# wei-zeng98/piano-a2s

Measured on AMD Instinct MI355X. Metric: training clips/sec (12 s, 5-bar), higher is better.
Workload: dtype f32

## Files before the change

piano_a2s_amd/csrc/a2s_api.hip:

```cpp
#include "a2s_common.h"
#include "../../include/a2s.h"

thread_local char a2s_err_msg[512] = {0};
long long a2s_launch_counter = 0;

int a2s_gemm_impl(hipStream_t, int, int, int, float, const float*, long, long, const float*, long, long, float, float*, long,
                  const float*, int, int, long, long, long, int, float*, size_t);
size_t a2s_gemm_workspace_bytes_impl(int, int, int, int);
int a2s_gemm_affine_impl(hipStream_t, int, int, int, float, const float*, long, long, const float*, long, long, float, float*, long, const float*,
                         int, int, long, long, long, int, float*, size_t, const float*, const float*, int, const float*, const float*, int,
                         const float*, const float*, const float*, const float*, const float*, float*, int, int, const float*, const float*);
int a2s_absmax_impl(hipStream_t, const float*, long, float*);
void a2s_gemm_f16x2_set(int);
int a2s_gemm_f16x2_enabled(void);
int a2s_gemm_bnstats_slots(int);
int a2s_conv3x3_impl(hipStream_t, const float*, const float*, float*, const float*, const float*, float*, int, int, int, int, int, int, float*,
                     const float*, const float*, const float*, const float*, const float*, const float*, const float*, float*);
void a2s_conv_rows_set(int);
void a2s_conv_c1_fast_set(int);
int a2s_conv_c1_fast_enabled(void);
int a2s_conv_rows_enabled(void);
void a2s_wgrad_rows_set(int);
int a2s_wgrad_rows_enabled(void);
void a2s_staff_emb_fast_set(int);
int a2s_staff_emb_fast_enabled(void);
void a2s_conv_f16x2_set(int);
int a2s_conv_f16x2_enabled(void);
size_t a2s_conv3x3_workspace_floats_impl(int);
void a2s_conv_bf16x3_set(int);
void a2s_gemm_split_set(int);
void a2s_wgrad_split_set(int);
int a2s_wgrad_split_enabled(void);
int a2s_gemm_split_enabled(void);
int a2s_conv_bf16x3_enabled(void);
int a2s_conv3x3_stat_blocks_impl(int, int, int, int);
int a2s_bn_finalize_impl(hipStream_t, const float*, int, int, double, const float*, const float*, float*, float*, long long*,
// ... 194 lines not shown
    if (!strcmp(key, "attn_deep")) { a2s_attn_deep_set(value); return A2S_OK; }
    if (!strcmp(key, "attn_defer_combine")) { a2s_attn_defer_combine_set(value); return A2S_OK; }
    if (!strcmp(key, "dec_mid")) { a2s_dec_mid_set(value); return A2S_OK; }
    if (!strcmp(key, "attn_pair")) { a2s_attn_pair_set(value); return A2S_OK; }
    if (!strcmp(key, "attn_pair_fused_rows")) { a2s_attn_pair_fused_rows_set(value); return A2S_OK; }
    if (!strcmp(key, "dec_fused_max_rows")) { a2s_dec_fused_max_rows_set(value); return A2S_OK; }
    if (!strcmp(key, "gru_fused")) { a2s_gru_step_fused_set(value); return A2S_OK; }
    if (!strcmp(key, "gru_persist")) { a2s_gru_persist_set(value); return A2S_OK; }
    if (!strcmp(key, "gru_persist_alone")) { a2s_gru_persist_alone_set(value); return A2S_OK; }
    if (!strcmp(key, "dec_persist")) { a2s_dec_persist_set(value); return A2S_OK; }
    if (!strcmp(key, "persist_force_agent")) { a2s_persist_dbg_set(PERSIST_DBG_FORCE_AGENT, value); return A2S_OK; }
    if (!strcmp(key, "persist_inject_abort")) { a2s_persist_dbg_set(PERSIST_DBG_INJECT_ABORT, value); return A2S_OK; }
    if (!strcmp(key, "gemm_tile")) { a2s_gemm_debug_tile_impl(value); return A2S_OK; }
    if (!strcmp(key, "conv_bf16x3")) { a2s_conv_bf16x3_set(value); return A2S_OK; }
    if (!strcmp(key, "conv_rows")) { a2s_conv_rows_set(value); return A2S_OK; }
    if (!strcmp(key, "conv_c1_fast")) { a2s_conv_c1_fast_set(value); return A2S_OK; }
    if (!strcmp(key, "wgrad_rows")) { a2s_wgrad_rows_set(value); return A2S_OK; }
    if (!strcmp(key, "staff_emb_fast")) { a2s_staff_emb_fast_set(value); return A2S_OK; }
    if (!strcmp(key, "conv_f16x2")) { a2s_conv_f16x2_set(value); return A2S_OK; }
    if (!strcmp(key, "wgrad_f16x2")) { a2s_wgrad_f16x2_set(value); return A2S_OK; }
    if (!strcmp(key, "gemm_bf16x3")) { a2s_gemm_split_set(value); return A2S_OK; }
    if (!strcmp(key, "gemm_f16x2")) { a2s_gemm_f16x2_set(value); return A2S_OK; }
    if (!strcmp(key, "wgrad_bf16x3")) { a2s_wgrad_split_set(value); return A2S_OK; }
    snprintf(a2s_err_msg, sizeof(a2s_err_msg), "a2s_debug_set: unknown key %s", key);
    return A2S_ERR_ARG;
}

int a2s_persist_abort_latch(void* device_word) { a2s_persist_latch_set(device_word); return A2S_OK; }

int a2s_debug_get(const char* key) {
    if (key && !strcmp(key, "attn_bulk_cap")) return a2s_attn_bulk_cap_enabled();
    if (key && !strcmp(key, "attn_deep")) return a2s_attn_deep_max_clips();
    if (key && !strcmp(key, "attn_defer_combine")) return a2s_attn_defer_combine_enabled();
    if (key && !strcmp(key, "dec_mid")) return a2s_dec_mid_enabled();
    if (key && !strcmp(key, "attn_pair")) return a2s_attn_pair_enabled();
    if (key && !strcmp(key, "attn_pair_fused_rows")) return a2s_attn_pair_fused_rows();
    if (key && !strcmp(key, "attn_pair_launches")) return (int)a2s_attn_pair_launches();
    if (key && !strcmp(key, "attn_pair_bwd_launches")) return (int)a2s_attn_pair_bwd_launches();
    if (key && !strcmp(key, "dec_mid_launches")) return a2s_dec_mid_launches();
    if (key && !strcmp(key, "conv_bf16x3")) return a2s_conv_bf16x3_enabled();
    if (key && !strcmp(key, "conv_rows")) return a2s_conv_rows_enabled();
    if (key && !strcmp(key, "conv_c1_fast")) return a2s_conv_c1_fast_enabled();
    if (key && !strcmp(key, "wgrad_rows")) return a2s_wgrad_rows_enabled();
    if (key && !strcmp(key, "staff_emb_fast")) return a2s_staff_emb_fast_enabled();
    if (key && !strcmp(key, "conv_f16x2")) return a2s_conv_f16x2_enabled();
    if (key && !strcmp(key, "wgrad_f16x2")) return a2s_wgrad_f16x2_enabled();
    if (key && !strcmp(key, "gemm_bf16x3")) return a2s_gemm_split_enabled();
    if (key && !strcmp(key, "gemm_f16x2")) return a2s_gemm_f16x2_enabled();
    if (key && !strcmp(key, "wgrad_bf16x3")) return a2s_wgrad_split_enabled();
    if (key && !strcmp(key, "gru_fused")) return a2s_gru_step_fused_enabled();
    if (key && !strcmp(key, "gru_persist")) return a2s_gru_persist_enabled();
    if (key && !strcmp(key, "gru_persist_alone")) return a2s_gru_persist_alone();
    if (key && !strcmp(key, "dec_persist")) return a2s_dec_persist_enabled();
    if (key && !strcmp(key, "dec_persist_launches")) return a2s_dec_persist_launches();
    if (key && !strcmp(key, "persist_force_agent")) return a2s_persist_dbg_get(PERSIST_DBG_FORCE_AGENT);
    if (key && !strcmp(key, "persist_inject_abort")) return a2s_persist_dbg_get(PERSIST_DBG_INJECT_ABORT);
// ... 254 lines not shown
```

piano_a2s_amd/csrc/a2s_conv_rows.hip:

```cpp
#include "a2s_common.h"
#include <type_traits>

#define RW_P 120
#define RW_SROW 288
#define RW_SLOTS 5
#ifndef RW_EB
#define RW_EB 4
#endif
#define RW_HDR 160

typedef short s16x4 __attribute__((ext_vector_type(4)));
typedef short s16x8 __attribute__((ext_vector_type(8)));
#define RW_LDS(p) ((__attribute__((address_space(3))) s16x4*)(p))

template <int CIN>
struct RwGeom {
    static constexpr int NB = CIN / 4;
    static constexpr int KS = (3 * NB + 7) / 8;
    static constexpr int TS = CIN * RW_SROW;
    static constexpr int SLOT = 2 * TS + (CIN % 8 ? 128 : 0);
    static constexpr int ITEMS = CIN * 32;
    static constexpr int XIT = (ITEMS + 255) / 256;
};

// ... 452 lines not shown
        const int grp = tid / (NJ * 5), c = tid % (NJ * 5);
        const float s = red[grp][c][0] + red[grp + 4][c][0], s2 = red[grp][c][1] + red[grp + 4][c][1];
        const float m = fmaxf(red[grp][c][2], red[grp + 4][c][2]);
        if (a.stat_partial) {
            a.stat_partial[((long)blockIdx.x * COUT + tid) * 2 + 0] = s;
            a.stat_partial[((long)blockIdx.x * COUT + tid) * 2 + 1] = s2;
        }
        if (a.out_absmax) {
            const unsigned bits = __float_as_uint(m);
            if (bits > __hip_atomic_load(reinterpret_cast<unsigned*>(a.out_absmax + tid), __ATOMIC_RELAXED, __HIP_MEMORY_SCOPE_AGENT))
                atomicMax(reinterpret_cast<unsigned*>(a.out_absmax + tid), bits);
        }
    }
}

template <int CIN, int COUT>
__global__ __launch_bounds__(256) void rows16_pack(const float* __restrict__ w, int flip, const float* __restrict__ in_scale,
                                                   const float* __restrict__ in_shift, const float* __restrict__ in_absmax,
                                                   const float* __restrict__ x_absmax, unsigned char* __restrict__ wimg, float* __restrict__ hdr,
                                                   float* __restrict__ out_absmax) {
    static_assert(COUT == 40, "rows16: 40 output channels");
    using G = RwGeom<CIN>;
    __shared__ int kci[CIN];
    __shared__ float red[16];
    __shared__ int kw[16];
    const int tile = blockIdx.x, tid = threadIdx.x;
    auto column = [&](int li, int& co, int& df) {
        if (tile < 6) { co = (tile / 3) * 16 + li; df = tile % 3; }
        else if (tile == 6) { co = 32 + (li & 7); df = li >> 3; }
        else { co = li < 8 ? 32 + li : -1; df = 2; }
    };
    if (tid < CIN) {
        int k = 0;
        if (in_scale) k = pow2_scale_exp(fabsf(in_scale[tid]) * (in_absmax ? in_absmax[tid] : 1.f) + fabsf(in_shift[tid]), 14);
        kci[tid] = k;
        if (tile == 0) {
            hdr[tid] = in_scale ? ldexpf(in_scale[tid], k) : 1.f;
            hdr[40 + tid] = in_scale ? ldexpf(in_shift[tid], k) : 0.f;
        }
    }
    if (tile == 0 && tid == 0) hdr[120] = ldexpf(1.f, (!in_scale && x_absmax) ? pow2_scale_exp(*x_absmax, 14) : 0);
    if (tile == 0 && out_absmax && tid < COUT) out_absmax[tid] = 0.f;
    __syncthreads();
// ... 21 lines not shown
        int co, df;
        column(li, co, df);
        float v = 0.f;
        if (co >= 0 && kb < 3 * G::NB) v = ldexpf(weight(co, 4 * (kb % G::NB) + e, (kb / G::NB) * 3 + df), kw[li]);
        unsigned t0, t1;
        split2_pair_f16(v, 0.f, t0, t1);
        unsigned short* dst = reinterpret_cast<unsigned short*>(wimg + ((size_t)(tile * G::KS + s) * 2) * 1024 + lane * 16 + e8 * 2);
        dst[0] = (unsigned short)t0;
        dst[512] = (unsigned short)t1;
    }
}

__device__ __forceinline__ float rw_ror8(float x) {
    return __int_as_float(__builtin_amdgcn_update_dpp(0, __float_as_int(x), 0x128, 0xf, 0xf, true));
}

#define R16_SLOTS 4
template <int CIN, int COUT, bool AFFINE, bool BNRED, bool PIPE = false>
__global__ __launch_bounds__(512, 2) void conv3x3_rows16(RowsArgs a) {
    static_assert(COUT == 40, "rows16: 40 output channels");
    using G = RwGeom<CIN>;
    constexpr int NTHR = 512, KS = G::KS;
    constexpr int XIT = (G::ITEMS + NTHR - 1) / NTHR;
    __shared__ __attribute__((aligned(16))) unsigned char ring[R16_SLOTS * G::SLOT];
    __shared__ __attribute__((aligned(16))) unsigned char b1img[PIPE ? 8 * G::KS * 1024 : 16];
    __shared__ float xch[2][5][2][16];
    __shared__ float red[8][16][3];
    __shared__ float tab[(AFFINE ? 2 * CIN : 0) + (BNRED ? 4 * COUT : 0) + 4];
    __shared__ __attribute__((aligned(16))) unsigned char dump[(G::ITEMS % NTHR) ? NTHR * 16 : 16];

    const int tid = threadIdx.x, lane = tid & 63;
    const int wave = __builtin_amdgcn_readfirstlane(tid >> 6);
    const int q = lane & 15, g = lane >> 4;
    const bool wide = wave < 4;
    const int m0 = wide ? 4 * (wave & 1) : 2 * (wave - 4);
    const int nm = wide ? 4 : 2;
    const int tile0 = wide ? 3 * (wave >> 1) : 6;
    const bool neg = wave & 1;
    const float sg = neg ? -1.f : 1.f;
    const int bnd_l = wide ? (wave & 1 ? (wave >> 1) : -1) : (wave > 4 ? wave - 3 : -1);
    const int bnd_r = wide ? (wave & 1 ? -1 : (wave >> 1)) : (wave < 7 ? wave - 2 : -1);

    int bid = blockIdx.x;
    {
        const int per = (int)gridDim.x / 8;
        if (bid < per * 8) bid = (bid % 8) * per + bid / 8;
    }
    const int ft = bid % a.tilesF; bid /= a.tilesF;
    const int strip = bid % a.nstrips, b = bid / a.nstrips;
    const int f_base = ft * RW_P;
    const int t_lo = strip * a.strip_len, t_hi = min(a.T, t_lo + a.strip_len);

    const unsigned sgn = neg ? 0x80008000u : 0u;
    constexpr int BWT = PIPE ? 1 : 2;
    s16x8 bw[3][KS][BWT];
#pragma unroll
    for (int d = 0; d < 3; ++d)
#pragma unroll
        for (int s = 0; s < KS; ++s)
#pragma unroll
            for (int tm = 0; tm < BWT; ++tm) {
                uint4 v = *reinterpret_cast<const uint4*>(a.wimg + ((size_t)((tile0 + ((wide || d < 2) ? d : 0)) * KS + s) * 2 + tm) * 1024 + lane * 16);
                v.x ^= sgn; v.y ^= sgn; v.z ^= sgn; v.w ^= sgn;
                bw[d][s][tm] = __builtin_bit_cast(s16x8, v);
            }
    if (PIPE) {
        for (int e = tid; e < 8 * KS * 64; e += NTHR)
            *reinterpret_cast<uint4*>(b1img + (size_t)e * 16) = *reinterpret_cast<const uint4*>(a.wimg + ((size_t)(e >> 6) * 2 + 1) * 1024 + (e & 63) * 16);
    }
    auto bterm1 = [&](int d, int s) -> s16x8 {
        if (PIPE) {
            uint4 v = *reinterpret_cast<const uint4*>(b1img + ((tile0 + ((wide || d < 2) ? d : 0)) * KS + s) * 1024 + lane * 16);
            v.x ^= sgn; v.y ^= sgn; v.z ^= sgn; v.w ^= sgn;
            return __builtin_bit_cast(s16x8, v);
        }
        return bw[d][s][BWT - 1];
    };
    const int co = wide ? (wave >> 1) * 16 + q : 32 + (q & 7);
    const bool useful = wide || q < 8;
    const float xscale = a.hdr[120];
    const float unsc = useful ? a.hdr[80 + co] / xscale * sg : 0.f;
    if (AFFINE && tid < 2 * CIN) tab[tid] = a.hdr[tid < CIN ? tid : 40 + tid - CIN];
    if (BNRED && tid < 4 * COUT) {
        const float* src = tid < COUT ? a.yl_mean : tid < 2 * COUT ? a.yl_invstd : tid < 3 * COUT ? a.yl_scale : a.yl_shift;
        tab[tid] = src[tid % COUT];
    }
    __syncthreads();
    float bm = 0.f, bi = 0.f, bsc = 0.f, bsh = 0.f;
    if (BNRED && useful) { bm = tab[co]; bi = tab[COUT + co]; bsc = tab[2 * COUT + co]; bsh = tab[3 * COUT + co]; }
    f32x2 st_s = {0.f, 0.f}, st_s2 = {0.f, 0.f};
    float st_m = 0.f;

    unsigned aaddr[KS][2];
#pragma unroll
// ... 43 lines not shown
        *reinterpret_cast<uint2*>(p0) = t0;
        *reinterpret_cast<uint2*>(p1) = t1;
    };

    f32x4 acc[4][3];
    auto multiply = [&](auto NMc, auto NTc, int crow, int cslot, const f32x4 (&xr)[XIT]) {
        constexpr int NM = decltype(NMc)::value, NT = decltype(NTc)::value;
        const bool cok = crow >= 0 && crow < a.T && colok;
        unsigned char* const cbase = ring + cslot * G::SLOT;
#pragma unroll
        for (int i = 0; i < NM; ++i)
#pragma unroll
            for (int d = 0; d < NT; ++d) acc[i][d] = (f32x4){0.f, 0.f, 0.f, 0.f};
#pragma unroll
        for (int s = 0; s < KS; ++s) {
#pragma unroll
            for (int ig = 0; ig < NM / 2; ++ig) {
                s16x8 av[2][2];
#pragma unroll
                for (int tm = 0; tm < 2; ++tm)
#pragma unroll
                    for (int ii = 0; ii < 2; ++ii) {
                        const int off = tm * G::TS + (ig * 2 + ii) * 32;
                        const s16x4 lo = __builtin_amdgcn_ds_read_tr16_b64_v4i16(RW_LDS(ring + aaddr[s][0] + off));
                        const s16x4 hi = __builtin_amdgcn_ds_read_tr16_b64_v4i16(RW_LDS(ring + aaddr[s][1] + off));
                        av[tm][ii] = __builtin_shufflevector(lo, hi, 0, 1, 2, 3, 4, 5, 6, 7);
                    }
#define R16_PRODUCT(TA, TB)                                                                                                  \
    _Pragma("unroll") for (int d = 0; d < NT; ++d)                                                                           \
        _Pragma("unroll") for (int ii = 0; ii < 2; ++ii)                                                                     \
            acc[ig * 2 + ii][d] = __builtin_amdgcn_mfma_f32_16x16x32_f16(__builtin_bit_cast(f16x8, av[TA][ii]), __builtin_bit_cast(f16x8, bw[d][s][TB < BWT ? TB : 0]), acc[ig * 2 + ii][d], 0, 0, 0);
                R16_PRODUCT(1, 0)
                R16_PRODUCT(0, 1)
                R16_PRODUCT(0, 0)
#undef R16_PRODUCT
            }
#pragma unroll
            for (int it = 0; it < XIT; ++it)
                if (it * KS / XIT == s) commit_item(it, cok, cbase, xr[it]);
        }
    };
    auto advance = [&]() {
#pragma unroll
        for (int s = 0; s < KS; ++s)
#pragma unroll
            for (int r = 0; r < 2; ++r) {
                const unsigned n = aaddr[s][r] + G::SLOT;
                aaddr[s][r] = min(n, n - R16_SLOTS * G::SLOT);
            }
    };

    const int up_addr = (((g + 3) & 3) * 16 + q) * 4;
    const int dn_addr = (((g + 1) & 3) * 16 + q) * 4;
    unsigned okbits = 0;
#pragma unroll
    for (int i = 0; i < 4; ++i) {
        const int p = 16 * (m0 + i) + 4 * g;
        if (useful && i < nm && p >= 4 && p < 4 + RW_P && f_base - 4 + p < a.F) okbits |= 1u << i;
    }
    const __amdgpu_buffer_rsrc_t yrsrc = __builtin_amdgcn_make_buffer_rsrc(a.y + (long)b * a.T * COUT * a.F, 0, (unsigned)((long)a.T * COUT * a.F * 4), 0x00020000);
    const __amdgpu_buffer_rsrc_t ylrsrc = __builtin_amdgcn_make_buffer_rsrc(const_cast<float*>(BNRED ? a.yl + (long)b * a.T * COUT * a.F : a.x), 0,
                                                                            BNRED ? (unsigned)((long)a.T * COUT * a.F * 4) : 0u, 0x00020000);
    const int yvo = (co * a.F + f_base - 4 + 16 * m0 + 4 * g) * 4;
    f32x4 ylv[BNRED ? 4 : 1];
    auto yl_fetch = [&](int t) {
        if (!BNRED) return;
        const int yrow_off = t * COUT * a.F * 4;
#pragma unroll
        for (int i = 0; i < 4; ++i)
            if (i < nm) ylv[BNRED ? i : 0] = __builtin_bit_cast(f32x4, __builtin_amdgcn_raw_buffer_load_b128(ylrsrc, yvo + 64 * i, yrow_off, 0));
    };
    auto epilogue = [&](auto WIDEc, int t, int par) {
        constexpr bool WIDE = decltype(WIDEc)::value;
        constexpr int NM = WIDE ? 4 : 2, D2 = WIDE ? 2 : 1;
        const int yrow_off = t * COUT * a.F * 4;
        const float xl = bnd_l >= 0 ? xch[par][bnd_l >= 0 ? bnd_l : 0][0][q] * sg : 0.f;
        const float xr_ = bnd_r >= 0 ? xch[par][bnd_r >= 0 ? bnd_r : 0][1][q] * sg : 0.f;
        unsigned ob = okbits;
        asm volatile("" : "+v"(ob));
        float X[NM], Y[NM];
#pragma unroll
        for (int i = 0; i < NM; ++i) {
            const float up_src = (g == 3) ? (i > 0 ? acc[i > 0 ? i - 1 : 0][0][3] : xl) : acc[i][0][3];
            const float dn_src = (g == 0) ? (i < NM - 1 ? acc[i < NM - 1 ? i + 1 : NM - 1][D2][0] : xr_) : acc[i][D2][0];
            X[i] = __int_as_float(__builtin_amdgcn_ds_bpermute(up_addr, __float_as_int(up_src)));
            Y[i] = __int_as_float(__builtin_amdgcn_ds_bpermute(dn_addr, __float_as_int(dn_src)));
        }
#pragma unroll
        for (int i = 0; i < NM; ++i) {
            const bool ok = ob >> i & 1;
            const float us = ok ? unsc : 0.f;
            f32x4 d1;
#pragma unroll
            for (int r = 0; r < 4; ++r) d1[r] = WIDE ? acc[i][1][r] : rw_ror8(acc[i][0][r]);
            f32x4 o;
            o[0] = ((X[i] + d1[0]) + acc[i][D2][1]) * us;
            o[1] = ((acc[i][0][0] + d1[1]) + acc[i][D2][2]) * us;
            o[2] = ((acc[i][0][1] + d1[2]) + acc[i][D2][3]) * us;
            o[3] = ((acc[i][0][2] + d1[3]) + Y[i]) * us;
            if (ok) __builtin_amdgcn_raw_buffer_store_b128(__builtin_bit_cast(u32x4, o), yrsrc, yvo + 64 * i, yrow_off, 0);
            if (BNRED) {
                const f32x4 xv = ylv[BNRED ? i : 0];
                f32x4 gm, xh;
#pragma unroll
                for (int k = 0; k < 4; ++k) {
                    gm[k] = (fmaf(xv[k], bsc, bsh) > 0.f) ? o[k] : 0.f;
                    xh[k] = fmaf(xv[k], bi, -bm * bi);
                }
                st_s += (f32x2){gm[0], gm[1]}; st_s += (f32x2){gm[2], gm[3]};
                st_s2 += (f32x2){gm[0], gm[1]} * (f32x2){xh[0], xh[1]}; st_s2 += (f32x2){gm[2], gm[3]} * (f32x2){xh[2], xh[3]};
                if (a.out_absmax) st_m = fmaxf(fmaxf(st_m, fmaxf(fabsf(o[0]), fabsf(o[1]))), fmaxf(fabsf(o[2]), fabsf(o[3])));
            } else {
                st_s += (f32x2){o[0], o[1]}; st_s += (f32x2){o[2], o[3]};
// ... 14 lines not shown
    __syncthreads();

    if constexpr (PIPE) {
        f32x4 accp[2][4][3];
#pragma unroll
        for (int e = 0; e < 2; ++e)
#pragma unroll
            for (int i = 0; i < 4; ++i)
#pragma unroll
                for (int d = 0; d < 3; ++d) accp[e][i][d] = (f32x4){0.f, 0.f, 0.f, 0.f};
        auto yl_tile = [&](int i, int t) -> f32x4 {
            return __builtin_bit_cast(f32x4, __builtin_amdgcn_raw_buffer_load_b128(ylrsrc, yvo + 64 * i, t * COUT * a.F * 4, 0));
        };
        auto epi_tile = [&](auto WIDEc, auto SETc, int i, int t, float xl, float xr_, unsigned ob, const f32x4& ylt) {
            constexpr bool WIDE = decltype(WIDEc)::value;
            constexpr int SET = decltype(SETc)::value, NM = WIDE ? 4 : 2, D2 = WIDE ? 2 : 1;
            const int yrow_off = t * COUT * a.F * 4;
            const float up_src = (g == 3) ? (i > 0 ? accp[SET][i > 0 ? i - 1 : 0][0][3] : xl) : accp[SET][i][0][3];
            const float dn_src = (g == 0) ? (i < NM - 1 ? accp[SET][i < NM - 1 ? i + 1 : NM - 1][D2][0] : xr_) : accp[SET][i][D2][0];
            const float X = __int_as_float(__builtin_amdgcn_ds_bpermute(up_addr, __float_as_int(up_src)));
            const float Y = __int_as_float(__builtin_amdgcn_ds_bpermute(dn_addr, __float_as_int(dn_src)));
            const bool ok = ob >> i & 1;
            const float us = ok ? unsc : 0.f;
            f32x4 d1;
#pragma unroll
            for (int r = 0; r < 4; ++r) d1[r] = WIDE ? accp[SET][i][1][r] : rw_ror8(accp[SET][i][0][r]);
            f32x4 o;
            o[0] = ((X + d1[0]) + accp[SET][i][D2][1]) * us;
            o[1] = ((accp[SET][i][0][0] + d1[1]) + accp[SET][i][D2][2]) * us;
            o[2] = ((accp[SET][i][0][1] + d1[2]) + accp[SET][i][D2][3]) * us;
            o[3] = ((accp[SET][i][0][2] + d1[3]) + Y) * us;
            if (ok) __builtin_amdgcn_raw_buffer_store_b128(__builtin_bit_cast(u32x4, o), yrsrc, yvo + 64 * i, yrow_off, 0);
            if (BNRED) {
                const f32x4 xv = ylt;
                f32x4 gm, xh;
#pragma unroll
                for (int k = 0; k < 4; ++k) {
                    gm[k] = (fmaf(xv[k], bsc, bsh) > 0.f) ? o[k] : 0.f;
                    xh[k] = fmaf(xv[k], bi, -bm * bi);
                }
                st_s += (f32x2){gm[0], gm[1]}; st_s += (f32x2){gm[2], gm[3]};
                st_s2 += (f32x2){gm[0], gm[1]} * (f32x2){xh[0], xh[1]}; st_s2 += (f32x2){gm[2], gm[3]} * (f32x2){xh[2], xh[3]};
                if (a.out_absmax) st_m = fmaxf(fmaxf(st_m, fmaxf(fabsf(o[0]), fabsf(o[1]))), fmaxf(fabsf(o[2]), fabsf(o[3])));
            } else {
                st_s += (f32x2){o[0], o[1]}; st_s += (f32x2){o[2], o[3]};
                st_s2 += (f32x2){o[0], o[1]} * (f32x2){o[0], o[1]}; st_s2 += (f32x2){o[2], o[3]} * (f32x2){o[2], o[3]};
                st_m = fmaxf(fmaxf(st_m, fmaxf(fabsf(o[0]), fabsf(o[1]))), fmaxf(fabsf(o[2]), fabsf(o[3])));
            }
        };
        auto multiply_p = [&](auto WIDEc, auto CURc, int t_e, int crow, int cslot, const f32x4 (&xr)[XIT]) {
            constexpr bool WIDE = decltype(WIDEc)::value;
            constexpr int CUR = decltype(CURc)::value, NM = WIDE ? 4 : 2, NT = WIDE ? 3 : 2;
            const bool cok = crow >= 0 && crow < a.T && colok;
            unsigned char* const cbase = ring + cslot * G::SLOT;
            const bool ev = t_e >= t_lo;
            const float xl = (ev && bnd_l >= 0) ? xch[1 - CUR][bnd_l >= 0 ? bnd_l : 0][0][q] * sg : 0.f;
            const float xr_ = (ev && bnd_r >= 0) ? xch[1 - CUR][bnd_r >= 0 ? bnd_r : 0][1][q] * sg : 0.f;
            unsigned ob = ev ? okbits : 0u;
            asm volatile("" : "+v"(ob));
#pragma unroll
            for (int i = 0; i < NM; ++i)
#pragma unroll
                for (int d = 0; d < NT; ++d) accp[CUR][i][d] = (f32x4){0.f, 0.f, 0.f, 0.f};
#pragma unroll
            for (int s = 0; s < KS; ++s) {
                f32x4 ylt[(BNRED && NM > KS) ? NM / KS : 1];
                if (BNRED) {
#pragma unroll
                    for (int i = 0; i < NM; ++i)
                        if (i * KS / NM == s) ylt[(NM > KS) ? i - s * NM / KS : 0] = (ev || true) ? yl_tile(i, t_e) : (f32x4){0.f, 0.f, 0.f, 0.f};
                }
                s16x8 b1[NT];
#pragma unroll
                for (int d = 0; d < NT; ++d) b1[d] = bterm1(d, s);
#pragma unroll
                for (int ig = 0; ig < NM / 2; ++ig) {
                    s16x8 av[2][2];
#pragma unroll
                    for (int tm = 0; tm < 2; ++tm)
#pragma unroll
                        for (int ii = 0; ii < 2; ++ii) {
                            const int off = tm * G::TS + (ig * 2 + ii) * 32;
                            const s16x4 lo = __builtin_amdgcn_ds_read_tr16_b64_v4i16(RW_LDS(ring + aaddr[s][0] + off));
                            const s16x4 hi = __builtin_amdgcn_ds_read_tr16_b64_v4i16(RW_LDS(ring + aaddr[s][1] + off));
                            av[tm][ii] = __builtin_shufflevector(lo, hi, 0, 1, 2, 3, 4, 5, 6, 7);
// ... 8 lines not shown
#undef R16P_PRODUCT
                }
#pragma unroll
                for (int it = 0; it < XIT; ++it)
                    if (it * KS / XIT == s) commit_item(it, cok, cbase, xr[it]);
#pragma unroll
                for (int i = 0; i < NM; ++i)
                    if (i * KS / NM == s) epi_tile(WIDEc, std::integral_constant<int, 1 - CUR>{}, i, t_e, xl, xr_, ob, ylt[(BNRED && NM > KS) ? i - s * NM / KS : 0]);
            }
        };
        int slot_w = 3;
        auto row = [&](auto CURc, int t) {
            constexpr int CUR = decltype(CURc)::value;
            if (wide) multiply_p(std::true_type{}, CURc, t - 1, t + 2, slot_w, xa);
            else multiply_p(std::false_type{}, CURc, t - 1, t + 2, slot_w, xa);
            if (bnd_r >= 0 && g == 3) xch[CUR][bnd_r >= 0 ? bnd_r : 0][0][q] = (wide ? accp[CUR][3][0][3] : accp[CUR][1][0][3]) * sg;
            if (bnd_l >= 0 && g == 0) xch[CUR][bnd_l >= 0 ? bnd_l : 0][1][q] = (wide ? accp[CUR][0][2][0] : accp[CUR][0][1][0]) * sg;
            __syncthreads();
            issue(t + 3, xa);
            slot_w = slot_w == R16_SLOTS - 1 ? 0 : slot_w + 1;
            advance();
        };
        using C0 = std::integral_constant<int, 0>; using C1 = std::integral_constant<int, 1>;
        int t = t_lo, last = 0;
        for (;;) {
            row(C0{}, t);
            if (++t >= t_hi) { last = 0; break; }
            row(C1{}, t);
            if (++t >= t_hi) { last = 1; break; }
        }
        {
            const float xl = bnd_l >= 0 ? xch[last][bnd_l >= 0 ? bnd_l : 0][0][q] * sg : 0.f;
// ... 4 lines not shown
            for (int i = 0; i < 4; ++i) {
                if (i < nm) {
                    const f32x4 ylt = BNRED ? yl_tile(i, t_hi - 1) : (f32x4){0.f, 0.f, 0.f, 0.f};
                    if (wide) { if (last) epi_tile(std::true_type{}, C1{}, i, t_hi - 1, xl, xr_, ob, ylt); else epi_tile(std::true_type{}, C0{}, i, t_hi - 1, xl, xr_, ob, ylt); }
                    else if (i < 2) { if (last) epi_tile(std::false_type{}, C1{}, i < 2 ? i : 0, t_hi - 1, xl, xr_, ob, ylt); else epi_tile(std::false_type{}, C0{}, i < 2 ? i : 0, t_hi - 1, xl, xr_, ob, ylt); }
                }
            }
        }
    } else {
    int slot_w = 3, par = 0;
#ifdef RW_TRACE
    const int rp = wave & 1, ng = wave >> 1;
    const int trace_first = (int)gridDim.x / 2;
    const int trace_wg = ((int)blockIdx.x >= trace_first && (int)blockIdx.x < trace_first + RW_TRACE_WGS) ? (int)blockIdx.x - trace_first : -1;
#endif
    using I2 = std::integral_constant<int, 2>; using I3 = std::integral_constant<int, 3>; using I4 = std::integral_constant<int, 4>;
    for (int t = t_lo; t < t_hi; ++t) {
#ifdef RW_TRACE
        const int trace_it = t - t_lo - 40;
#endif
        RW_STAMP(0);
        yl_fetch(t);
        if (wide) multiply(I4{}, I3{}, t + 2, slot_w, xa);
        else multiply(I2{}, I2{}, t + 2, slot_w, xa);
        RW_STAMP(1);
        if (bnd_r >= 0 && g == 3) xch[par][bnd_r >= 0 ? bnd_r : 0][0][q] = (wide ? acc[3][0][3] : acc[1][0][3]) * sg;
        if (bnd_l >= 0 && g == 0) xch[par][bnd_l >= 0 ? bnd_l : 0][1][q] = (wide ? acc[0][2][0] : acc[0][1][0]) * sg;
        __syncthreads();
        RW_STAMP(2);
        if (wide) epilogue(std::true_type{}, t, par);
        else epilogue(std::false_type{}, t, par);
        RW_STAMP(3);
        issue(t + 3, xa);
        RW_STAMP(4);
        slot_w = slot_w == R16_SLOTS - 1 ? 0 : slot_w + 1;
        par ^= 1;
        advance();
    }
    }

    {
        float s = st_s[0] + st_s[1], s2 = st_s2[0] + st_s2[1], m = st_m;
        s += __shfl_xor(s, 16, 64); s2 += __shfl_xor(s2, 16, 64); m = fmaxf(m, __shfl_xor(m, 16, 64));
        s += __shfl_xor(s, 32, 64); s2 += __shfl_xor(s2, 32, 64); m = fmaxf(m, __shfl_xor(m, 32, 64));
        if (g == 0) { red[wave][q][0] = s; red[wave][q][1] = s2; red[wave][q][2] = m; }
    }
    __syncthreads();
    if (tid < COUT) {
        float s = 0.f, s2 = 0.f, m = 0.f;
        const int w0 = tid < 32 ? 2 * (tid >> 4) : 4, nw = tid < 32 ? 2 : 4, c = tid < 32 ? tid & 15 : tid - 32;
        for (int k = 0; k < nw; ++k) { s += red[w0 + k][c][0]; s2 += red[w0 + k][c][1]; m = fmaxf(m, red[w0 + k][c][2]); }
        if (a.stat_partial) {
            a.stat_partial[((long)blockIdx.x * COUT + tid) * 2 + 0] = s;
            a.stat_partial[((long)blockIdx.x * COUT + tid) * 2 + 1] = s2;
        }
        if (a.out_absmax) {
            const unsigned bits = __float_as_uint(m);
            if (bits > __hip_atomic_load(reinterpret_cast<unsigned*>(a.out_absmax + tid), __ATOMIC_RELAXED, __HIP_MEMORY_SCOPE_AGENT))
                atomicMax(reinterpret_cast<unsigned*>(a.out_absmax + tid), bits);
        }
    }
}

static int g_conv_rows = -1;
void a2s_conv_rows_set(int on) { g_conv_rows = on; }
int a2s_conv_rows_enabled(void) {
    if (g_conv_rows < 0) { const char* e = getenv("A2S_CONV_ROWS"); g_conv_rows = e ? atoi(e) : 7; }
    return g_conv_rows;
}
bool a2s_conv_rows_eligible(int F, int Cin) { return a2s_conv_rows_enabled() && F % 4 == 0 && (Cin == 20 || Cin == 40); }

static void rows_geometry(int B, int T, int F, int* tilesF, int* nstrips, int* strip_len) {
    *tilesF = a2s_cdiv(F, RW_P);
    int ns = a2s_cdiv(2048, (long)B * *tilesF);
    ns = ns < 1 ? 1 : ns;
    const int max_ns = T / 16 > 1 ? T / 16 : 1;
    ns = ns > max_ns ? max_ns : ns;
    int len = a2s_cdiv(T, ns);
    len += len & 1;
    *strip_len = len;
    *nstrips = a2s_cdiv(T, len);
}
int a2s_conv_rows_blocks(int B, int T, int F) {
    int tf, ns, len;
    rows_geometry(B, T, F, &tf, &ns, &len);
    return B * tf * ns;
}
size_t a2s_conv_rows_workspace_floats(int Cin) {
    return (size_t)9 * RwGeom<40>::KS * 2 * 1024 / 4 + RW_HDR + 64;
}

template <int CIN, int COUT>
static int rows16_launch(hipStream_t st, const RowsArgs& a, bool affine, bool bnred, int nwork) {
    constexpr int NT = 512;
    const int en = a2s_conv_rows_enabled();
    if (affine && (en & 4)) hipLaunchKernelGGL((conv3x3_rows16<CIN, COUT, true, false, true>), dim3(nwork), dim3(NT), 0, st, a);
    else if (affine) hipLaunchKernelGGL((conv3x3_rows16<CIN, COUT, true, false>), dim3(nwork), dim3(NT), 0, st, a);
    else if (bnred && (en & 8)) hipLaunchKernelGGL((conv3x3_rows16<CIN, COUT, false, true, true>), dim3(nwork), dim3(NT), 0, st, a);
    else if (bnred) hipLaunchKernelGGL((conv3x3_rows16<CIN, COUT, false, true>), dim3(nwork), dim3(NT), 0, st, a);
    else hipLaunchKernelGGL((conv3x3_rows16<CIN, COUT, false, false>), dim3(nwork), dim3(NT), 0, st, a);
    A2S_CHECK_LAUNCH("conv3x3_rows16");
    return A2S_OK;
}
template <int CIN, int COUT>
static int rows_launch(hipStream_t st, const RowsArgs& a, bool affine, bool bnred, int nwork) {
    if (affine) hipLaunchKernelGGL((conv3x3_rows<CIN, COUT, true, false>), dim3(nwork), dim3(512), 0, st, a);
    else if (bnred) hipLaunchKernelGGL((conv3x3_rows<CIN, COUT, false, true>), dim3(nwork), dim3(512), 0, st, a);
    else hipLaunchKernelGGL((conv3x3_rows<CIN, COUT, false, false>), dim3(nwork), dim3(512), 0, st, a);
    A2S_CHECK_LAUNCH("conv3x3_rows");
    return A2S_OK;
}
template <int CIN, int COUT>
static void rows_pack_launch(hipStream_t st, const float* w, int flip, const float* in_scale, const float* in_shift, const float* in_absmax,
                             const float* x_absmax, unsigned char* wimg, float* hdr, float* out_absmax) {
    hipLaunchKernelGGL((rows_pack<CIN, COUT>), dim3(COUT / 5), dim3(256), 0, st, w, flip, in_scale, in_shift, in_absmax, x_absmax, wimg, hdr, out_absmax);
}

int a2s_absmax_impl(hipStream_t, const float*, long, float*);

int a2s_conv3x3_rows_impl(hipStream_t st, const float* x, const float* w, float* y, const float* in_scale, const float* in_shift,
                          const float* in_absmax, float* stat_partial, float* out_absmax, int B, int T, int F, int Cin, int Cout, int flip,
                          float* ws, const float* yl, const float* yl_mean, const float* yl_invstd, const float* yl_scale, const float* yl_shift,
                          const float* x_absmax) {
    A2S_REQUIRE(F % 4 == 0 && (Cin == 20 || Cin == 40) && (Cout == 20 || Cout == 40), "conv3x3_rows: unsupported shape F=%d Cin=%d Cout=%d", F, Cin, Cout);
    A2S_REQUIRE(!(in_scale && yl), "conv3x3_rows: input affine and BatchNorm-backward statistics are exclusive");
    if (yl && Cin == 20 && Cout == 20 && out_absmax) {
        const int rc = a2s_conv3x3_rows_impl(st, x, w, y, in_scale, in_shift, in_absmax, stat_partial, nullptr, B, T, F, Cin, Cout, flip, ws, yl, yl_mean, yl_invstd,
                                             yl_scale, yl_shift, x_absmax);
        return rc != A2S_OK ? rc : a2s_channel_absmax_impl(st, y, (long)B * T, Cout, F, out_absmax);
    }
    unsigned char* wimg = reinterpret_cast<unsigned char*>(ws);
    float* hdr = ws + (size_t)9 * RwGeom<40>::KS * 2 * 1024 / 4;
    float* scratch = hdr + RW_HDR;
    if (in_scale && !in_absmax) {
        const int rc = a2s_channel_absmax_impl(st, x, (long)B * T, Cin, F, scratch);
        if (rc != A2S_OK) return rc;
        in_absmax = scratch;
    }
    if (!in_scale && !x_absmax) {
        const int rc = a2s_absmax_impl(st, x, (long)B * T * Cin * F, scratch);
        if (rc != A2S_OK) return rc;
        x_absmax = scratch;
    }
    RowsArgs a{x, y, wimg, hdr, stat_partial, out_absmax, yl, yl_mean, yl_invstd, yl_scale, yl_shift, B, T, F, 0, 0, 0, 0};
    rows_geometry(B, T, F, &a.tilesF, &a.nstrips, &a.strip_len);
    a.nwork = B * a.tilesF * a.nstrips;
    const bool affine = in_scale != nullptr, bnred = yl != nullptr;
#define R16_CASE(CI, CO)                                                                                                     \
    if (Cin == CI && Cout == CO && (a2s_conv_rows_enabled() & 2)) {                                                          \
        hipLaunchKernelGGL((rows16_pack<CI, CO>), dim3(8), dim3(256), 0, st, w, flip, in_scale, in_shift, in_absmax, x_absmax, wimg, hdr, out_absmax); \
        A2S_CHECK_LAUNCH("rows16_pack");                                                                                     \
        return rows16_launch<CI, CO>(st, a, affine, bnred, a.nwork);                                                         \
    }
    R16_CASE(20, 40) R16_CASE(40, 40)
#undef R16_CASE
#define RW_CASE(CI, CO)                                                                                                      \
    if (Cin == CI && Cout == CO) {                                                                                           \
        rows_pack_launch<CI, CO>(st, w, flip, in_scale, in_shift, in_absmax, x_absmax, wimg, hdr, out_absmax);               \
        A2S_CHECK_LAUNCH("rows_pack");                                                                                       \
        return rows_launch<CI, CO>(st, a, affine, bnred, a.nwork);                                                           \
    }
    RW_CASE(20, 20) RW_CASE(20, 40) RW_CASE(40, 40) RW_CASE(40, 20)
#undef RW_CASE
    A2S_FAIL(A2S_ERR_ARG, "conv3x3_rows: no instance for %d -> %d", Cin, Cout);
}
```

Measured before the change: 607.7.

## Extend rows16 MFMA conv kernel to 20-output-channel convolutions

```diff
diff --git a/piano_a2s_amd/csrc/a2s_api.hip b/piano_a2s_amd/csrc/a2s_api.hip
--- a/piano_a2s_amd/csrc/a2s_api.hip
+++ b/piano_a2s_amd/csrc/a2s_api.hip
@@ -20,6 +20,8 @@
 void a2s_conv_c1_fast_set(int);
 int a2s_conv_c1_fast_enabled(void);
 int a2s_conv_rows_enabled(void);
+void a2s_conv_rows16_c20_set(int);
+int a2s_conv_rows16_c20_enabled(void);
 void a2s_wgrad_rows_set(int);
 int a2s_wgrad_rows_enabled(void);
 void a2s_staff_emb_fast_set(int);
@@ -244,6 +246,7 @@
     if (!strcmp(key, "gemm_tile")) { a2s_gemm_debug_tile_impl(value); return A2S_OK; }
     if (!strcmp(key, "conv_bf16x3")) { a2s_conv_bf16x3_set(value); return A2S_OK; }
     if (!strcmp(key, "conv_rows")) { a2s_conv_rows_set(value); return A2S_OK; }
+    if (!strcmp(key, "conv_rows16_c20")) { a2s_conv_rows16_c20_set(value); return A2S_OK; }
     if (!strcmp(key, "conv_c1_fast")) { a2s_conv_c1_fast_set(value); return A2S_OK; }
     if (!strcmp(key, "wgrad_rows")) { a2s_wgrad_rows_set(value); return A2S_OK; }
     if (!strcmp(key, "staff_emb_fast")) { a2s_staff_emb_fast_set(value); return A2S_OK; }
@@ -270,6 +273,7 @@
     if (key && !strcmp(key, "dec_mid_launches")) return a2s_dec_mid_launches();
     if (key && !strcmp(key, "conv_bf16x3")) return a2s_conv_bf16x3_enabled();
     if (key && !strcmp(key, "conv_rows")) return a2s_conv_rows_enabled();
+    if (key && !strcmp(key, "conv_rows16_c20")) return a2s_conv_rows16_c20_enabled();
     if (key && !strcmp(key, "conv_c1_fast")) return a2s_conv_c1_fast_enabled();
     if (key && !strcmp(key, "wgrad_rows")) return a2s_wgrad_rows_enabled();
     if (key && !strcmp(key, "staff_emb_fast")) return a2s_staff_emb_fast_enabled();
diff --git a/piano_a2s_amd/csrc/a2s_conv_rows.hip b/piano_a2s_amd/csrc/a2s_conv_rows.hip
--- a/piano_a2s_amd/csrc/a2s_conv_rows.hip
+++ b/piano_a2s_amd/csrc/a2s_conv_rows.hip
@@ -490,19 +490,24 @@
     }
 }
 
+template <int COUT>
+constexpr int rows16_tiles() { return COUT == 40 ? 8 : 4; }
 template <int CIN, int COUT>
 __global__ __launch_bounds__(256) void rows16_pack(const float* __restrict__ w, int flip, const float* __restrict__ in_scale,
                                                    const float* __restrict__ in_shift, const float* __restrict__ in_absmax,
                                                    const float* __restrict__ x_absmax, unsigned char* __restrict__ wimg, float* __restrict__ hdr,
                                                    float* __restrict__ out_absmax) {
-    static_assert(COUT == 40, "rows16: 40 output channels");
+    static_assert(COUT == 40 || COUT == 20, "rows16: 40 or 20 output channels");
     using G = RwGeom<CIN>;
     __shared__ int kci[CIN];
     __shared__ float red[16];
     __shared__ int kw[16];
     const int tile = blockIdx.x, tid = threadIdx.x;
     auto column = [&](int li, int& co, int& df) {
-        if (tile < 6) { co = (tile / 3) * 16 + li; df = tile % 3; }
+        if (COUT == 20) {
+            if (tile < 3) { co = li; df = tile; }
+            else { co = li < 12 ? 16 + (li & 3) : -1; df = li >> 2; }
+        } else if (tile < 6) { co = (tile / 3) * 16 + li; df = tile % 3; }
         else if (tile == 6) { co = 32 + (li & 7); df = li >> 3; }
         else { co = li < 8 ? 32 + li : -1; df = 2; }
     };
@@ -554,17 +559,25 @@
 __device__ __forceinline__ float rw_ror8(float x) {
     return __int_as_float(__builtin_amdgcn_update_dpp(0, __float_as_int(x), 0x128, 0xf, 0xf, true));
 }
+__device__ __forceinline__ float rw_rol4(float x) {
+    return __int_as_float(__builtin_amdgcn_update_dpp(0, __float_as_int(x), 0x12c, 0xf, 0xf, true));
+}
 
 #define R16_SLOTS 4
 template <int CIN, int COUT, bool AFFINE, bool BNRED, bool PIPE = false>
-__global__ __launch_bounds__(512, 2) void conv3x3_rows16(RowsArgs a) {
-    static_assert(COUT == 40, "rows16: 40 output channels");
+__global__ __launch_bounds__(512, (CIN == 20 && COUT == 20 && !PIPE) ? 4 : 2) void conv3x3_rows16(RowsArgs a) {
+    static_assert(COUT == 40 || COUT == 20, "rows16: 40 or 20 output channels");
     using G = RwGeom<CIN>;
     constexpr int NTHR = 512, KS = G::KS;
     constexpr int XIT = (G::ITEMS + NTHR - 1) / NTHR;
+    constexpr bool C20 = COUT == 20;
+    constexpr int NMW = C20 ? 2 : 4;
+    constexpr int NTN = C20 ? 1 : 2;
+    constexpr int NBND = C20 ? 6 : 5;
+    constexpr bool B1LDS = PIPE || (CIN == 20 && C20);
     __shared__ __attribute__((aligned(16))) unsigned char ring[R16_SLOTS * G::SLOT];
-    __shared__ __attribute__((aligned(16))) unsigned char b1img[PIPE ? 8 * G::KS * 1024 : 16];
-    __shared__ float xch[2][5][2][16];
+    __shared__ __attribute__((aligned(16))) unsigned char b1img[B1LDS ? rows16_tiles<COUT>() * G::KS * 1024 : 16];
+    __shared__ float xch[2][NBND][2][16];
     __shared__ float red[8][16][3];
     __shared__ float tab[(AFFINE ? 2 * CIN : 0) + (BNRED ? 4 * COUT : 0) + 4];
     __shared__ __attribute__((aligned(16))) unsigned char dump[(G::ITEMS % NTHR) ? NTHR * 16 : 16];
@@ -573,13 +586,15 @@
     const int wave = __builtin_amdgcn_readfirstlane(tid >> 6);
     const int q = lane & 15, g = lane >> 4;
     const bool wide = wave < 4;
-    const int m0 = wide ? 4 * (wave & 1) : 2 * (wave - 4);
-    const int nm = wide ? 4 : 2;
-    const int tile0 = wide ? 3 * (wave >> 1) : 6;
+    const int m0 = (wide && !C20) ? 4 * (wave & 1) : 2 * (wave & 3);
+    const int nm = wide ? NMW : 2;
+    const int tile0 = C20 ? (wide ? 0 : 3) : (wide ? 3 * (wave >> 1) : 6);
     const bool neg = wave & 1;
     const float sg = neg ? -1.f : 1.f;
-    const int bnd_l = wide ? (wave & 1 ? (wave >> 1) : -1) : (wave > 4 ? wave - 3 : -1);
-    const int bnd_r = wide ? (wave & 1 ? -1 : (wave >> 1)) : (wave < 7 ? wave - 2 : -1);
+    const int bnd_l = C20 ? ((wave & 3) ? 3 * (wave >> 2) + (wave & 3) - 1 : -1)
+                          : wide ? (wave & 1 ? (wave >> 1) : -1) : (wave > 4 ? wave - 3 : -1);
+    const int bnd_r = C20 ? ((wave & 3) < 3 ? 3 * (wave >> 2) + (wave & 3) : -1)
+                          : wide ? (wave & 1 ? -1 : (wave >> 1)) : (wave < 7 ? wave - 2 : -1);
 
     int bid = blockIdx.x;
     {
@@ -592,7 +607,7 @@
     const int t_lo = strip * a.strip_len, t_hi = min(a.T, t_lo + a.strip_len);
 
     const unsigned sgn = neg ? 0x80008000u : 0u;
-    constexpr int BWT = PIPE ? 1 : 2;
+    constexpr int BWT = B1LDS ? 1 : 2;
     s16x8 bw[3][KS][BWT];
 #pragma unroll
     for (int d = 0; d < 3; ++d)
@@ -600,24 +615,24 @@
         for (int s = 0; s < KS; ++s)
 #pragma unroll
             for (int tm = 0; tm < BWT; ++tm) {
-                uint4 v = *reinterpret_cast<const uint4*>(a.wimg + ((size_t)((tile0 + ((wide || d < 2) ? d : 0)) * KS + s) * 2 + tm) * 1024 + lane * 16);
+                uint4 v = *reinterpret_cast<const uint4*>(a.wimg + ((size_t)((tile0 + ((wide || d < NTN) ? d : 0)) * KS + s) * 2 + tm) * 1024 + lane * 16);
                 v.x ^= sgn; v.y ^= sgn; v.z ^= sgn; v.w ^= sgn;
                 bw[d][s][tm] = __builtin_bit_cast(s16x8, v);
             }
-    if (PIPE) {
-        for (int e = tid; e < 8 * KS * 64; e += NTHR)
+    if (B1LDS) {
+        for (int e = tid; e < rows16_tiles<COUT>() * KS * 64; e += NTHR)
             *reinterpret_cast<uint4*>(b1img + (size_t)e * 16) = *reinterpret_cast<const uint4*>(a.wimg + ((size_t)(e >> 6) * 2 + 1) * 1024 + (e & 63) * 16);
     }
     auto bterm1 = [&](int d, int s) -> s16x8 {
-        if (PIPE) {
-            uint4 v = *reinterpret_cast<const uint4*>(b1img + ((tile0 + ((wide || d < 2) ? d : 0)) * KS + s) * 1024 + lane * 16);
+        if (B1LDS) {
+            uint4 v = *reinterpret_cast<const uint4*>(b1img + ((tile0 + ((wide || d < NTN) ? d : 0)) * KS + s) * 1024 + lane * 16);
             v.x ^= sgn; v.y ^= sgn; v.z ^= sgn; v.w ^= sgn;
             return __builtin_bit_cast(s16x8, v);
         }
         return bw[d][s][BWT - 1];
     };
-    const int co = wide ? (wave >> 1) * 16 + q : 32 + (q & 7);
-    const bool useful = wide || q < 8;
+    const int co = C20 ? (wide ? q : 16 + (q & 3)) : (wide ? (wave >> 1) * 16 + q : 32 + (q & 7));
+    const bool useful = wide || q < (C20 ? 4 : 8);
     const float xscale = a.hdr[120];
     const float unsc = useful ? a.hdr[80 + co] / xscale * sg : 0.f;
     if (AFFINE && tid < 2 * CIN) tab[tid] = a.hdr[tid < CIN ? tid : 40 + tid - CIN];
@@ -691,6 +706,9 @@
             for (int d = 0; d < NT; ++d) acc[i][d] = (f32x4){0.f, 0.f, 0.f, 0.f};
 #pragma unroll
         for (int s = 0; s < KS; ++s) {
+            s16x8 b1[NT];
+#pragma unroll
+            for (int d = 0; d < NT; ++d) b1[d] = bterm1(d, s);
 #pragma unroll
             for (int ig = 0; ig < NM / 2; ++ig) {
                 s16x8 av[2][2];
@@ -703,13 +721,13 @@
                         const s16x4 hi = __builtin_amdgcn_ds_read_tr16_b64_v4i16(RW_LDS(ring + aaddr[s][1] + off));
                         av[tm][ii] = __builtin_shufflevector(lo, hi, 0, 1, 2, 3, 4, 5, 6, 7);
                     }
-#define R16_PRODUCT(TA, TB)                                                                                                  \
+#define R16_PRODUCT(TA, BV)                                                                                                  \
     _Pragma("unroll") for (int d = 0; d < NT; ++d)                                                                           \
         _Pragma("unroll") for (int ii = 0; ii < 2; ++ii)                                                                     \
-            acc[ig * 2 + ii][d] = __builtin_amdgcn_mfma_f32_16x16x32_f16(__builtin_bit_cast(f16x8, av[TA][ii]), __builtin_bit_cast(f16x8, bw[d][s][TB < BWT ? TB : 0]), acc[ig * 2 + ii][d], 0, 0, 0);
-                R16_PRODUCT(1, 0)
-                R16_PRODUCT(0, 1)
-                R16_PRODUCT(0, 0)
+            acc[ig * 2 + ii][d] = __builtin_amdgcn_mfma_f32_16x16x32_f16(__builtin_bit_cast(f16x8, av[TA][ii]), __builtin_bit_cast(f16x8, BV), acc[ig * 2 + ii][d], 0, 0, 0);
+                R16_PRODUCT(1, bw[d][s][0])
+                R16_PRODUCT(0, b1[d])
+                R16_PRODUCT(0, bw[d][s][0])
 #undef R16_PRODUCT
             }
 #pragma unroll
@@ -728,7 +746,7 @@
     };
 
     const int up_addr = (((g + 3) & 3) * 16 + q) * 4;
-    const int dn_addr = (((g + 1) & 3) * 16 + q) * 4;
+    const int dn_addr = (((g + 1) & 3) * 16 + ((C20 && !wide) ? (q + 8) & 15 : q)) * 4;
     unsigned okbits = 0;
 #pragma unroll
     for (int i = 0; i < 4; ++i) {
@@ -749,7 +767,7 @@
     };
     auto epilogue = [&](auto WIDEc, int t, int par) {
         constexpr bool WIDE = decltype(WIDEc)::value;
-        constexpr int NM = WIDE ? 4 : 2, D2 = WIDE ? 2 : 1;
+        constexpr int NM = WIDE ? NMW : 2, D2 = WIDE ? 2 : NTN - 1;
         const int yrow_off = t * COUT * a.F * 4;
         const float xl = bnd_l >= 0 ? xch[par][bnd_l >= 0 ? bnd_l : 0][0][q] * sg : 0.f;
         const float xr_ = bnd_r >= 0 ? xch[par][bnd_r >= 0 ? bnd_r : 0][1][q] * sg : 0.f;
@@ -767,13 +785,16 @@
         for (int i = 0; i < NM; ++i) {
             const bool ok = ob >> i & 1;
             const float us = ok ? unsc : 0.f;
-            f32x4 d1;
-#pragma unroll
-            for (int r = 0; r < 4; ++r) d1[r] = WIDE ? acc[i][1][r] : rw_ror8(acc[i][0][r]);
+            f32x4 d1, d2;
+#pragma unroll
+            for (int r = 0; r < 4; ++r) {
+                d1[r] = WIDE ? acc[i][1][r] : C20 ? rw_rol4(acc[i][0][r]) : rw_ror8(acc[i][0][r]);
+                d2[r] = (!WIDE && C20) ? rw_ror8(acc[i][0][r]) : acc[i][D2][r];
+            }
             f32x4 o;
-            o[0] = ((X[i] + d1[0]) + acc[i][D2][1]) * us;
-            o[1] = ((acc[i][0][0] + d1[1]) + acc[i][D2][2]) * us;
-            o[2] = ((acc[i][0][1] + d1[2]) + acc[i][D2][3]) * us;
+            o[0] = ((X[i] + d1[0]) + d2[1]) * us;
+            o[1] = ((acc[i][0][0] + d1[1]) + d2[2]) * us;
+            o[2] = ((acc[i][0][1] + d1[2]) + d2[3]) * us;
             o[3] = ((acc[i][0][2] + d1[3]) + Y[i]) * us;
             if (ok) __builtin_amdgcn_raw_buffer_store_b128(__builtin_bit_cast(u32x4, o), yrsrc, yvo + 64 * i, yrow_off, 0);
             if (BNRED) {
@@ -818,7 +839,7 @@
         };
         auto epi_tile = [&](auto WIDEc, auto SETc, int i, int t, float xl, float xr_, unsigned ob, const f32x4& ylt) {
             constexpr bool WIDE = decltype(WIDEc)::value;
-            constexpr int SET = decltype(SETc)::value, NM = WIDE ? 4 : 2, D2 = WIDE ? 2 : 1;
+            constexpr int SET = decltype(SETc)::value, NM = WIDE ? NMW : 2, D2 = WIDE ? 2 : NTN - 1;
             const int yrow_off = t * COUT * a.F * 4;
             const float up_src = (g == 3) ? (i > 0 ? accp[SET][i > 0 ? i - 1 : 0][0][3] : xl) : accp[SET][i][0][3];
             const float dn_src = (g == 0) ? (i < NM - 1 ? accp[SET][i < NM - 1 ? i + 1 : NM - 1][D2][0] : xr_) : accp[SET][i][D2][0];
@@ -826,13 +847,16 @@
             const float Y = __int_as_float(__builtin_amdgcn_ds_bpermute(dn_addr, __float_as_int(dn_src)));
             const bool ok = ob >> i & 1;
             const float us = ok ? unsc : 0.f;
-            f32x4 d1;
-#pragma unroll
-            for (int r = 0; r < 4; ++r) d1[r] = WIDE ? accp[SET][i][1][r] : rw_ror8(accp[SET][i][0][r]);
+            f32x4 d1, d2;
+#pragma unroll
+            for (int r = 0; r < 4; ++r) {
+                d1[r] = WIDE ? accp[SET][i][1][r] : C20 ? rw_rol4(accp[SET][i][0][r]) : rw_ror8(accp[SET][i][0][r]);
+                d2[r] = (!WIDE && C20) ? rw_ror8(accp[SET][i][0][r]) : accp[SET][i][D2][r];
+            }
             f32x4 o;
-            o[0] = ((X + d1[0]) + accp[SET][i][D2][1]) * us;
-            o[1] = ((accp[SET][i][0][0] + d1[1]) + accp[SET][i][D2][2]) * us;
-            o[2] = ((accp[SET][i][0][1] + d1[2]) + accp[SET][i][D2][3]) * us;
+            o[0] = ((X + d1[0]) + d2[1]) * us;
+            o[1] = ((accp[SET][i][0][0] + d1[1]) + d2[2]) * us;
+            o[2] = ((accp[SET][i][0][1] + d1[2]) + d2[3]) * us;
             o[3] = ((accp[SET][i][0][2] + d1[3]) + Y) * us;
             if (ok) __builtin_amdgcn_raw_buffer_store_b128(__builtin_bit_cast(u32x4, o), yrsrc, yvo + 64 * i, yrow_off, 0);
             if (BNRED) {
@@ -854,7 +878,7 @@
         };
         auto multiply_p = [&](auto WIDEc, auto CURc, int t_e, int crow, int cslot, const f32x4 (&xr)[XIT]) {
             constexpr bool WIDE = decltype(WIDEc)::value;
-            constexpr int CUR = decltype(CURc)::value, NM = WIDE ? 4 : 2, NT = WIDE ? 3 : 2;
+            constexpr int CUR = decltype(CURc)::value, NM = WIDE ? NMW : 2, NT = WIDE ? 3 : NTN;
             const bool cok = crow >= 0 && crow < a.T && colok;
             unsigned char* const cbase = ring + cslot * G::SLOT;
             const bool ev = t_e >= t_lo;
@@ -872,7 +896,7 @@
                 if (BNRED) {
 #pragma unroll
                     for (int i = 0; i < NM; ++i)
-                        if (i * KS / NM == s) ylt[(NM > KS) ? i - s * NM / KS : 0] = (ev || true) ? yl_tile(i, t_e) : (f32x4){0.f, 0.f, 0.f, 0.f};
+                        if (i * KS / NM == s) ylt[(NM > KS) ? i - s * NM / KS : 0] = yl_tile(i, ev ? t_e : t_lo);
                 }
                 s16x8 b1[NT];
 #pragma unroll
@@ -911,8 +935,8 @@
             constexpr int CUR = decltype(CURc)::value;
             if (wide) multiply_p(std::true_type{}, CURc, t - 1, t + 2, slot_w, xa);
             else multiply_p(std::false_type{}, CURc, t - 1, t + 2, slot_w, xa);
-            if (bnd_r >= 0 && g == 3) xch[CUR][bnd_r >= 0 ? bnd_r : 0][0][q] = (wide ? accp[CUR][3][0][3] : accp[CUR][1][0][3]) * sg;
-            if (bnd_l >= 0 && g == 0) xch[CUR][bnd_l >= 0 ? bnd_l : 0][1][q] = (wide ? accp[CUR][0][2][0] : accp[CUR][0][1][0]) * sg;
+            if (bnd_r >= 0 && g == 3) xch[CUR][bnd_r >= 0 ? bnd_r : 0][0][q] = (wide ? accp[CUR][NMW - 1][0][3] : accp[CUR][1][0][3]) * sg;
+            if (bnd_l >= 0 && g == 0) xch[CUR][bnd_l >= 0 ? bnd_l : 0][1][q] = (wide ? accp[CUR][0][2][0] : accp[CUR][0][NTN - 1][0]) * sg;
             __syncthreads();
             issue(t + 3, xa);
             slot_w = slot_w == R16_SLOTS - 1 ? 0 : slot_w + 1;
@@ -947,18 +971,19 @@
     const int trace_first = (int)gridDim.x / 2;
     const int trace_wg = ((int)blockIdx.x >= trace_first && (int)blockIdx.x < trace_first + RW_TRACE_WGS) ? (int)blockIdx.x - trace_first : -1;
 #endif
-    using I2 = std::integral_constant<int, 2>; using I3 = std::integral_constant<int, 3>; using I4 = std::integral_constant<int, 4>;
+    using I2 = std::integral_constant<int, 2>; using I3 = std::integral_constant<int, 3>;
+    using IMW = std::integral_constant<int, NMW>; using ITN = std::integral_constant<int, NTN>;
     for (int t = t_lo; t < t_hi; ++t) {
 #ifdef RW_TRACE
         const int trace_it = t - t_lo - 40;
 #endif
         RW_STAMP(0);
         yl_fetch(t);
-        if (wide) multiply(I4{}, I3{}, t + 2, slot_w, xa);
-        else multiply(I2{}, I2{}, t + 2, slot_w, xa);
+        if (wide) multiply(IMW{}, I3{}, t + 2, slot_w, xa);
+        else multiply(I2{}, ITN{}, t + 2, slot_w, xa);
         RW_STAMP(1);
-        if (bnd_r >= 0 && g == 3) xch[par][bnd_r >= 0 ? bnd_r : 0][0][q] = (wide ? acc[3][0][3] : acc[1][0][3]) * sg;
-        if (bnd_l >= 0 && g == 0) xch[par][bnd_l >= 0 ? bnd_l : 0][1][q] = (wide ? acc[0][2][0] : acc[0][1][0]) * sg;
+        if (bnd_r >= 0 && g == 3) xch[par][bnd_r >= 0 ? bnd_r : 0][0][q] = (wide ? acc[NMW - 1][0][3] : acc[1][0][3]) * sg;
+        if (bnd_l >= 0 && g == 0) xch[par][bnd_l >= 0 ? bnd_l : 0][1][q] = (wide ? acc[0][2][0] : acc[0][NTN - 1][0]) * sg;
         __syncthreads();
         RW_STAMP(2);
         if (wide) epilogue(std::true_type{}, t, par);
@@ -981,7 +1006,8 @@
     __syncthreads();
     if (tid < COUT) {
         float s = 0.f, s2 = 0.f, m = 0.f;
-        const int w0 = tid < 32 ? 2 * (tid >> 4) : 4, nw = tid < 32 ? 2 : 4, c = tid < 32 ? tid & 15 : tid - 32;
+        const int w0 = C20 ? (tid < 16 ? 0 : 4) : tid < 32 ? 2 * (tid >> 4) : 4, nw = (C20 || tid >= 32) ? 4 : 2;
+        const int c = C20 ? (tid < 16 ? tid : tid - 16) : tid < 32 ? tid & 15 : tid - 32;
         for (int k = 0; k < nw; ++k) { s += red[w0 + k][c][0]; s2 += red[w0 + k][c][1]; m = fmaxf(m, red[w0 + k][c][2]); }
         if (a.stat_partial) {
             a.stat_partial[((long)blockIdx.x * COUT + tid) * 2 + 0] = s;
@@ -1001,6 +1027,10 @@
     if (g_conv_rows < 0) { const char* e = getenv("A2S_CONV_ROWS"); g_conv_rows = e ? atoi(e) : 7; }
     return g_conv_rows;
 }
+static int g_conv_rows16_c20 = 1;
+void a2s_conv_rows16_c20_set(int on) { g_conv_rows16_c20 = on; }
+int a2s_conv_rows16_c20_enabled(void) { return g_conv_rows16_c20; }
+static bool rows16_selected(int Cout) { return (a2s_conv_rows_enabled() & 2) && (Cout == 40 || g_conv_rows16_c20); }
 bool a2s_conv_rows_eligible(int F, int Cin) { return a2s_conv_rows_enabled() && F % 4 == 0 && (Cin == 20 || Cin == 40); }
 
 static void rows_geometry(int B, int T, int F, int* tilesF, int* nstrips, int* strip_len) {
@@ -1026,7 +1056,7 @@
 template <int CIN, int COUT>
 static int rows16_launch(hipStream_t st, const RowsArgs& a, bool affine, bool bnred, int nwork) {
     constexpr int NT = 512;
-    const int en = a2s_conv_rows_enabled();
+    const int en = COUT == 20 ? 8 : a2s_conv_rows_enabled();
     if (affine && (en & 4)) hipLaunchKernelGGL((conv3x3_rows16<CIN, COUT, true, false, true>), dim3(nwork), dim3(NT), 0, st, a);
     else if (affine) hipLaunchKernelGGL((conv3x3_rows16<CIN, COUT, true, false>), dim3(nwork), dim3(NT), 0, st, a);
     else if (bnred && (en & 8)) hipLaunchKernelGGL((conv3x3_rows16<CIN, COUT, false, true, true>), dim3(nwork), dim3(NT), 0, st, a);
@@ -1057,7 +1087,7 @@
                           const float* x_absmax) {
     A2S_REQUIRE(F % 4 == 0 && (Cin == 20 || Cin == 40) && (Cout == 20 || Cout == 40), "conv3x3_rows: unsupported shape F=%d Cin=%d Cout=%d", F, Cin, Cout);
     A2S_REQUIRE(!(in_scale && yl), "conv3x3_rows: input affine and BatchNorm-backward statistics are exclusive");
-    if (yl && Cin == 20 && Cout == 20 && out_absmax) {
+    if (yl && Cin == 20 && Cout == 20 && out_absmax && !rows16_selected(Cout)) {
         const int rc = a2s_conv3x3_rows_impl(st, x, w, y, in_scale, in_shift, in_absmax, stat_partial, nullptr, B, T, F, Cin, Cout, flip, ws, yl, yl_mean, yl_invstd,
                                              yl_scale, yl_shift, x_absmax);
         return rc != A2S_OK ? rc : a2s_channel_absmax_impl(st, y, (long)B * T, Cout, F, out_absmax);
@@ -1080,12 +1110,12 @@
     a.nwork = B * a.tilesF * a.nstrips;
     const bool affine = in_scale != nullptr, bnred = yl != nullptr;
 #define R16_CASE(CI, CO)                                                                                                     \
-    if (Cin == CI && Cout == CO && (a2s_conv_rows_enabled() & 2)) {                                                          \
-        hipLaunchKernelGGL((rows16_pack<CI, CO>), dim3(8), dim3(256), 0, st, w, flip, in_scale, in_shift, in_absmax, x_absmax, wimg, hdr, out_absmax); \
+    if (Cin == CI && Cout == CO && rows16_selected(CO)) {                                                                    \
+        hipLaunchKernelGGL((rows16_pack<CI, CO>), dim3(rows16_tiles<CO>()), dim3(256), 0, st, w, flip, in_scale, in_shift, in_absmax, x_absmax, wimg, hdr, out_absmax); \
         A2S_CHECK_LAUNCH("rows16_pack");                                                                                     \
         return rows16_launch<CI, CO>(st, a, affine, bnred, a.nwork);                                                         \
     }
-    R16_CASE(20, 40) R16_CASE(40, 40)
+    R16_CASE(20, 40) R16_CASE(40, 40) R16_CASE(20, 20) R16_CASE(40, 20)
 #undef R16_CASE
 #define RW_CASE(CI, CO)                                                                                                      \
     if (Cin == CI && Cout == CO) {                                                                                           \
```

New measurement: 611.2, median of 6. About the same (+0.6%).
